# caspervdw/clustertracking

Measured on AMD Instinct MI355X. Metric: cluster-fits/sec, higher is better.
Workload: dtype f64

## Files before the change

clustertracking_amd/_lib.py:

```python
import collections
import contextlib
import ctypes as C
import os
import threading

from . import _abi

_HERE = os.path.dirname(os.path.abspath(__file__))
LIB_PATH = os.environ.get('CTREFINE_LIB') or os.path.join(_HERE, 'csrc', 'libctrefine.so')

_P = C.POINTER
_H = _S = C.c_void_p


def _stage(desc):
    return (C.c_int, [_H, _P(desc), _S])


SIGNATURES = {
    'ctr_abi_version': (C.c_int, []),
    'ctr_create': (C.c_int, [_P(C.c_void_p), C.c_int]),
    'ctr_destroy': (None, [_H]),
    'ctr_last_error': (C.c_char_p, [_H]),
    'ctr_validate_problem': (C.c_int, [_P(_abi.Problem), C.c_char_p, C.c_int]),
    'ctr_cluster_n_vars': (C.c_int, [_P(_abi.Problem), C.c_int]),
    'ctr_cluster_kernel': (C.c_int, [_P(_abi.Problem), C.c_int64, _P(_abi.KernelChoice)]),
    'ctr_refine_batch': (C.c_int, [_H, _P(_abi.Problem), _P(_abi.Batch)]),
    'ctr_plan_create': (C.c_int, [_H, _P(_abi.Problem), C.c_int64, C.c_void_p, _P(C.c_void_p)]),
    'ctr_plan_destroy': (None, [C.c_void_p]),
    'ctr_plan_tail': (C.c_int, [C.c_void_p, _P(C.c_int32), _P(C.c_int32), _P(C.c_int32)]),
    'ctr_refine_batch_device': (C.c_int, [_H, C.c_void_p, _P(_abi.Batch), _S]),
    'ctr_frame_max_device': (C.c_int, [_H, C.c_void_p, C.c_int32, C.c_int64, C.c_int64, C.c_void_p, _S]),
    'ctr_synchronize': (C.c_int, [_H, _S]),
    'ctr_last_kernel_ms': (C.c_int, [_H, _P(C.c_double), _P(C.c_double)]),
    'ctr_find_clusters': (C.c_int, [_H, C.c_int32, C.c_void_p, C.c_void_p, C.c_int64, C.c_void_p,
                                    C.c_void_p, C.c_void_p]),
    'ctr_engine_wait_stream': (C.c_int, [_H, _S]),
    'ctr_stream_wait_engine': (C.c_int, [_H, _S]),
    'ctr_draw_frames_device': (C.c_int, [_H, _P(_abi.Synth), C.c_void_p, _S]),
    'ctr_locate_maxima_device': _stage(_abi.Locate),
    'ctr_characterize_device': _stage(_abi.Characterize),
    'ctr_link_device': _stage(_abi.Link),
    'ctr_preprocess_device': _stage(_abi.Preprocess),
    'ctr_orientation_device': _stage(_abi.Orientation),
    'ctr_diffusion_device': _stage(_abi.Diffusion),
    'ctr_relocate_device': _stage(_abi.Relocate),
    'ctr_relocate_plan': (C.c_int, [_P(_abi.Relocate), _P(C.c_int64), _P(C.c_int64)]),
    'ctr_find_link_device': _stage(_abi.FindLink),
    'ctr_refine_com_device': _stage(_abi.RefineCom),
    'ctr_train_device': _stage(_abi.Train),
    'ctr_cluster_tracks_device': _stage(_abi.ClusterTracks),
    'ctr_cluster_tracks_plan': (C.c_int, [_P(_abi.ClusterTracks), _P(C.c_int64), _P(C.c_int32), _P(C.c_int32)]),
    'ctr_track_positions_device': _stage(_abi.TrackPositions),
    'ctr_drift_device': _stage(_abi.Drift),
    'ctr_drift_subtract_device': _stage(_abi.DriftSubtract),
    'ctr_filter_stubs_device': _stage(_abi.FilterStubs),
    'ctr_msd_device': _stage(_abi.Msd),
    'ctr_emsd_device': _stage(_abi.Emsd),
    'ctr_vanhove_device': _stage(_abi.Vanhove),
    'ctr_pair_correlation_device': _stage(_abi.PairCorrelation),
    'ctr_neighbors_device': _stage(_abi.Neighbors),
    'ctr_twopoint_device': _stage(_abi.TwoPoint),
    'ctr_shape_device': _stage(_abi.Shape),
    'ctr_shape_dynamics_device': _stage(_abi.ShapeDynamics),
    'ctr_shape_plan': (C.c_int, [_P(_abi.ShapeDynamics), _P(C.c_int32), _P(C.c_int32), _P(C.c_int64), _P(C.c_int64),
                                 _P(C.c_int64)]),
    'ctr_shape_histogram_device': _stage(_abi.ShapeHistogram),
    'ctr_residual_device': _stage(_abi.Residual),
    'ctr_residual_plan': (C.c_int, [_P(_abi.Residual), _P(C.c_int32), _P(C.c_int32), _P(C.c_int64), _P(C.c_int64),
                                    _P(C.c_int64), _P(C.c_int64)]),
    'ctr_fit_error_device': _stage(_abi.FitError),
    'ctr_fit_error_plan': (C.c_int, [_P(_abi.FitError), _P(C.c_int32), _P(C.c_int32), _P(C.c_int64), _P(C.c_int64),
                                     _P(C.c_int64)]),
    'ctr_contacts_device': _stage(_abi.Contacts),
    'ctr_contacts_plan': (C.c_int, [_P(_abi.Contacts), _P(C.c_int64), _P(C.c_int64), _P(C.c_int64)]),
    'ctr_refine_prepare_device': _stage(_abi.RefinePrepare),
    'ctr_refine_prepare_plan': (C.c_int, [_P(_abi.RefinePrepare), _P(C.c_int64)]),
    'ctr_find_link_refine_device': (C.c_int, [_H, _P(_abi.FindLink), _P(_abi.RefineCom), _S]),
    'ctr_diffusion_ci_device': _stage(_abi.DiffusionCI),
    'ctr_diffusion_ci_plan': (C.c_int, [_P(_abi.DiffusionCI), _P(C.c_int32), _P(C.c_int64), _P(C.c_int64),
                                        _P(C.c_int64)]),
    'ctr_set_stage_max_grid': (C.c_int32, [_H, C.c_int32]),
    'ctr_set_lane_limit': (C.c_int32, [C.c_int32, C.c_int32]),
# ... 135 lines not shown
    return ContactsPlan(scratch.value, tuple(tiles), tuple(grids))


def refine_prepare_plan(desc):
    return _plan('ctr_refine_prepare_plan', desc, C.c_int64())[0]


class Engine(object):

    def __init__(self, device=0):
        self._lib = load()
        self._h = C.c_void_p()
        rc = self._lib.ctr_create(C.byref(self._h), int(device))
        if rc != _abi.OK:
            msg = self._lib.ctr_last_error(None)
            self._h = None
            raise EngineError("ctr_create(device=%d) failed (%d): %s" % (
                device, rc, (msg or b'').decode()))
        self.device = int(device)

    def close(self):
        if getattr(self, '_h', None):
            self._lib.ctr_destroy(self._h)
            self._h = None

    __del__ = close

    def _check(self, rc, what, too_large=False):
        if rc != _abi.OK:
            msg = (self._lib.ctr_last_error(self._h) or b'').decode()
            if rc == _abi.ERR_INVALID:
                raise ValueError("%s: %s" % (what, msg))
            if rc == _abi.ERR_UNSUPPORTED and too_large:
                raise EngineError("%s: %s" % (what, msg))
            if rc == _abi.ERR_UNSUPPORTED:
                raise NotImplementedError("%s: %s" % (what, msg))
            raise EngineError("%s failed (%d): %s" % (what, rc, msg))

    def refine_batch(self, problem, batch):
        b = batch.as_struct()
        self._check(self._lib.ctr_refine_batch(self._h, C.byref(problem), C.byref(b)),
                    'ctr_refine_batch')
        return batch

    def plan(self, problem, feat_offset_host):
        import numpy as np
        off = np.ascontiguousarray(feat_offset_host, dtype=np.int32)
        plan = C.c_void_p()
        self._check(self._lib.ctr_plan_create(self._h, C.byref(problem), len(off) - 1,
                                              off.ctypes.data, C.byref(plan)),
                    'ctr_plan_create')
        return Plan(self._lib, plan)

    def refine_batch_device(self, plan, batch_struct, stream=None):
        self._check(self._lib.ctr_refine_batch_device(
            self._h, plan._p, C.byref(batch_struct), C.c_void_p(stream or 0)),
            'ctr_refine_batch_device')

    def frame_max_device(self, frames_ptr, dtype_code, n_frames, frame_elems, out_ptr,
                         stream=None):
        self._check(self._lib.ctr_frame_max_device(
            self._h, C.c_void_p(frames_ptr), dtype_code, n_frames, frame_elems,
            C.c_void_p(out_ptr), C.c_void_p(stream or 0)), 'ctr_frame_max_device')

    def find_clusters(self, pos, frame_offset, separation):
        import numpy as np
        pos = np.ascontiguousarray(pos, dtype=np.float64)
        off = np.ascontiguousarray(frame_offset, dtype=np.int32)
        sep = np.ascontiguousarray(separation, dtype=np.float64)
        n, nd = pos.shape
        labels = np.empty(n, dtype=np.int32)
        sizes = np.empty(n, dtype=np.int32)
        self._check(self._lib.ctr_find_clusters(self._h, nd, pos.ctypes.data, off.ctypes.data,
                                                len(off) - 1, sep.ctypes.data,
                                                labels.ctypes.data, sizes.ctypes.data),
                    'ctr_find_clusters')
        return labels, sizes

    def draw_frames_device(self, synth, frames_ptr, stream=None):
        self._check(self._lib.ctr_draw_frames_device(self._h, C.byref(synth), C.c_void_p(frames_ptr),
                                                     C.c_void_p(stream or 0)), 'ctr_draw_frames_device')

    def query_done(self):
        rc = self._lib.ctr_query_done(self._h)
        if rc < 0:
            raise EngineError("ctr_query_done failed: %s" % (self._lib.ctr_last_error(self._h) or b'').decode())
        return rc == 1

    def set_stage_max_grid(self, max_grid):
        return int(self._lib.ctr_set_stage_max_grid(self._h, C.c_int32(int(max_grid))))

    @contextlib.contextmanager
    def stage_max_grid(self, max_grid):
        before = self.set_stage_max_grid(max_grid)
        if before < 0:
            raise ValueError("stage_max_grid: %r is outside [0, 65536]" % (max_grid,))
        try:
            yield self
        finally:
            self.set_stage_max_grid(before)

    def set_lane_limit(self, n):
        return int(self._lib.ctr_set_lane_limit(C.c_int32(self.device), C.c_int32(int(n))))

    def synchronize(self, stream=None):
        self._check(self._lib.ctr_synchronize(self._h, C.c_void_p(stream or 0)),
# ... 65 lines not shown
    method.__doc__ = "``%s``: ``desc`` is its ``_abi`` descriptor with device pointers." % symbol
    return method


for _name, _symbol, _too_large in (
        ('locate_maxima_device', 'ctr_locate_maxima_device', True),
        ('characterize_device', 'ctr_characterize_device', False),
        ('link_device', 'ctr_link_device', False),
        ('preprocess_device', 'ctr_preprocess_device', True),
        ('orientation_device', 'ctr_orientation_device', False),
        ('diffusion_device', 'ctr_diffusion_device', False),
        ('diffusion_ci_device', 'ctr_diffusion_ci_device', False),
        ('relocate_device', 'ctr_relocate_device', False),
        ('find_link_device', 'ctr_find_link_device', False),
        ('refine_com_device', 'ctr_refine_com_device', False),
        ('train_device', 'ctr_train_device', False),
        ('cluster_tracks_device', 'ctr_cluster_tracks_device', False),
        ('track_positions_device', 'ctr_track_positions_device', False),
        ('drift_device', 'ctr_drift_device', False),
        ('drift_subtract_device', 'ctr_drift_subtract_device', False),
        ('filter_stubs_device', 'ctr_filter_stubs_device', False),
        ('msd_device', 'ctr_msd_device', False),
        ('emsd_device', 'ctr_emsd_device', False),
        ('vanhove_device', 'ctr_vanhove_device', False),
        ('pair_correlation_device', 'ctr_pair_correlation_device', False),
        ('neighbors_device', 'ctr_neighbors_device', False),
        ('twopoint_device', 'ctr_twopoint_device', False),
        ('shape_device', 'ctr_shape_device', False),
        ('shape_dynamics_device', 'ctr_shape_dynamics_device', False),
        ('shape_histogram_device', 'ctr_shape_histogram_device', False),
        ('residual_device', 'ctr_residual_device', False),
        ('contacts_device', 'ctr_contacts_device', False),
        ('fit_error_device', 'ctr_fit_error_device', False),
        ('refine_prepare_device', 'ctr_refine_prepare_device', False)):
    setattr(Engine, _name, _stage_method(_symbol, _too_large))


class Plan(object):
    def __init__(self, lib, p):
        self._lib, self._p = lib, p

    def close(self):
        if self._p:
            self._lib.ctr_plan_destroy(self._p)
            self._p = None

    def tail(self):
        fused, cap, grid = C.c_int32(), C.c_int32(), C.c_int32()
        rc = self._lib.ctr_plan_tail(self._p, C.byref(fused), C.byref(cap), C.byref(grid))
        if rc != _abi.OK:
            raise ValueError("ctr_plan_tail: no plan (%d)" % rc)
        return bool(fused.value), int(cap.value), int(grid.value)

    __del__ = close


_default_engines = {}


def default_engine(device=0):
    eng = _default_engines.get(device)
    if eng is None:
        eng = _default_engines[device] = Engine(device)
    return eng
```

clustertracking_amd/csrc/ctrefine.hip:

```cpp
#include <hip/hip_runtime.h>

#include <cmath>
#include <cstdio>
#include <cstdlib>
#include <cstring>
#include <algorithm>
#include <chrono>
#include <functional>
#include <map>
#include <mutex>
#include <string>
#include <vector>

#include "kargs.h"
#include "lane_sched.h"

namespace {

#include "device_common.h"
#include "stage_common.h"
#include "aux_kernels.h"
#include "synth_kernels.h"


std::string g_create_error;
std::mutex g_mutex;

}

constexpr int BIN_TOO_LARGE = MAXNT, BIN_SMALL1 = MAXNT + 1, BIN_SMALL2 = MAXNT + 2, BIN_LARGE = MAXNT + 3,
              BIN_CONS1 = MAXNT + 4, BIN_CONS2 = MAXNT + 5, NBINS = MAXNT + 6;
static_assert(NBINS <= 16, "FrontArgs (aux_kernels.h) holds 16 bins");
constexpr int NFAM = CTR_KFAM_LARGE_LOWPASS + 1, NSLOT = MAXNT + 2;
constexpr int SLOT_SINGLES8 = 0, SLOT_SINGLES64 = 1, SLOT_PAIRS64 = 2, SLOT_PAIRS16 = 3;
constexpr int64_t NARROW_WINDOW = 600;
constexpr int GATE_US = 20;
constexpr int LAUNCH_PAIRS16 = NBINS, LAUNCH_TAIL = NBINS + 1, NLAUNCH = NBINS + 2;
constexpr int TAIL_CAP = 256;
constexpr int TAIL_BINS[TAIL_SEGMENTS] = {BIN_SMALL2, 0, 1};

constexpr int TIMING_EVERY = 8;
struct LaunchTiming {
  lane_sched::Estimate est;
  hipEvent_t t0 = nullptr, t1 = nullptr;
  bool pending = false;
  int untimed = 0;
};

struct ctr_plan {
  ctr_problem prob;
  int64_t n_clusters = 0;
  int device = 0;
  int32_t* d_order = nullptr;
  int* d_front = nullptr;
  double* d_ws = nullptr;
  long long* d_ws_off = nullptr;
  mutable int large_epoch = 0;
  mutable LaunchTiming timing[NLAUNCH];
  int64_t bin_begin[NBINS + 1] = {0};
  int64_t bin_count[NBINS] = {0};
  int32_t bin_family[NBINS] = {0};
  int32_t bin_slot[NBINS] = {0};
  bool gate = false;
  bool pairs_split = false;
  bool tail_fused = false;
  int tail_grid = 0;
  int large_workgroups = 0;
  bool lowpass = false;
  double* d_lp_w = nullptr;
  int lp_half[3] = {0, 0, 0};
};

struct Scratch {
  void* ptr = nullptr;
  size_t bytes = 0;
  hipEvent_t event = nullptr;
};

struct LanePool {
  int device = 0, refs = 0;
  std::mutex mu;
  std::vector<hipStream_t> lanes;
  lane_sched::Pool books;
  std::vector<hipEvent_t> spare;
  explicit LanePool(int n) : books(n) {}
};

struct ctr_handle {
  int device = 0;
  hipStream_t stream = nullptr;
  LanePool* pool = nullptr;
  bool pending = false;
  bool own_dirty = false;
  hipEvent_t ev[4] = {nullptr, nullptr, nullptr, nullptr};
  bool ev_valid = false;
  std::string err;
  Scratch buf, enc, fmax;
  struct { KernelInfo k; bool attr_set; } kernels[NFAM][2][2][NSLOT] = {};
  KernelInfo tail[2] = {};
  bool tail_attr_set[2] = {false, false};
  hipEvent_t ev_done = nullptr;
  hipEvent_t ev_fork = nullptr, ev_gate = nullptr, ev_order = nullptr, ev_own = nullptr;
  int* d_counter = nullptr;
  Scratch link, motion;
  Scratch train;
  Scratch tracks;
  Scratch prepare;
  Scratch drift;
  Scratch msd;
  Scratch pcf;
  Scratch nbr;
  Scratch twopt;
  Scratch shape;
  Scratch resid;
  Scratch contacts;
  Scratch fiterr;
  unsigned stage_max_grid = STAGE_MAX_GRID;
};

namespace {

int fail(ctr_handle* h, int code, const std::string& msg) {
  if (h) h->err = msg;
  else { std::lock_guard<std::mutex> g(g_mutex); g_create_error = msg; }
  return code;
}

#define HIP_TRY(h, call)                                                                   \
  do {                                                                                     \
    hipError_t e_ = (call);                                                                \
    if (e_ != hipSuccess)                                                                  \
      return fail(h, CTR_ERR_DEVICE, std::string(#call) + ": " + hipGetErrorString(e_));   \
  } while (0)

std::map<int, LanePool*> g_pools;
std::mutex g_pool_mutex;

constexpr unsigned PROBE_US = 1000;
bool on_new_queue(const std::vector<hipStream_t>& lanes, hipStream_t cand) {
  for (int rep = 0; rep < 3; ++rep) {
    for (hipStream_t st : lanes) (void)hipStreamSynchronize(st);
    (void)hipStreamSynchronize(cand);
    for (hipStream_t st : lanes) hipLaunchKernelGGL(delay_kernel, dim3(1), dim3(WAVE), 0, st, (unsigned long long)PROBE_US * 100ull);
    const auto t0 = std::chrono::steady_clock::now();
    hipLaunchKernelGGL(delay_kernel, dim3(1), dim3(WAVE), 0, cand, (unsigned long long)PROBE_US * 100ull);
    bool ok = hipGetLastError() == hipSuccess;
    ok = hipStreamSynchronize(cand) == hipSuccess && ok;
    const double us = std::chrono::duration<double, std::micro>(std::chrono::steady_clock::now() - t0).count();
    for (hipStream_t st : lanes) ok = hipStreamSynchronize(st) == hipSuccess && ok;
    if (!ok) return true;
    if (us < 1.5 * PROBE_US) return true;
  }
  return false;
// ... 393 lines not shown
  std::string msg;
  int rc = validate(p, msg);
  if (rc) return fail(h, rc, msg);
  if (n_clusters < 0 || (n_clusters > 0 && !feat_offset_host)) return fail(h, CTR_ERR_INVALID, "bad cluster table");
  if (n_clusters > 0x7ffffff0LL) return fail(h, CTR_ERR_INVALID, "too many clusters for one batch");
  std::vector<int32_t> bin_of((size_t)n_clusters);
  ctr_plan* plan = new ctr_plan();
  plan->prob = *p;
  plan->n_clusters = n_clusters;
  plan->device = h->device;
  plan->lowpass = lowpass_of(p);
  std::vector<long long> ws_off((size_t)n_clusters, 0);
  long long ws_total = 0;
  const long long box_cap = window_volume(p);
  int npf = 0, nsh = 0;
  for (int k2 = 0; k2 < p->n_params; ++k2) {
    if (p->modes[k2] == CTR_MODE_VAR) ++npf;
    else if (p->modes[k2] != CTR_MODE_CONST) ++nsh;
  }
  for (int64_t c = 0; c < n_clusters; ++c) {
    const int64_t n = (int64_t)feat_offset_host[c + 1] - feat_offset_host[c];
    if (n < 0) { delete plan; return fail(h, CTR_ERR_INVALID, "feat_offset must be non-decreasing"); }
    const KernelChoice kc = choose_kernel(p, n);
    const int bin = kc.bin;
    if (bin == BIN_LARGE) {
      ws_off[(size_t)c] = ws_total;
      ws_total += large_ws((int)n, npf, nsh, box_cap).total;
    }
    if (plan->bin_count[bin] == 0) { plan->bin_family[bin] = kc.family; plan->bin_slot[bin] = kc.slot; }
    else if (plan->bin_family[bin] != kc.family || plan->bin_slot[bin] != kc.slot) {
      delete plan;
      return fail(h, CTR_ERR_INVALID, "internal: clusters of one bin with different kernels");
    }
    bin_of[(size_t)c] = bin;
    plan->bin_count[bin]++;
  }
  plan->bin_begin[0] = 0;
  for (int b = 0; b < NBINS; ++b) plan->bin_begin[b + 1] = plan->bin_begin[b] + plan->bin_count[b];
  const bool throughput = (p->flags & CTR_FLAG_THROUGHPUT) != 0;
  plan->gate = n_clusters > plan->bin_count[BIN_SMALL1] + plan->bin_count[BIN_SMALL2] + plan->bin_count[BIN_TOO_LARGE];
  plan->pairs_split = throughput && plan->bin_count[BIN_SMALL2] >= 64 && box_cap <= NARROW_WINDOW;
  {
    int nonempty = 0;
    bool family_ok = true;
    for (int sgm = 0; sgm < TAIL_SEGMENTS; ++sgm) {
      const int bin = TAIL_BINS[sgm];
      if (plan->bin_count[bin] == 0) continue;
      ++nonempty;
      if (bin < MAXNT && plan->bin_family[bin] != CTR_KFAM_GAUSS_TP) family_ok = false;
      plan->tail_grid += (int)std::min<int64_t>(plan->bin_count[bin], TAIL_CAP);
    }
    plan->tail_fused = throughput && p->ndim == 2 && !plan->lowpass && family_ok && nonempty >= 2;
    if (!plan->tail_fused) plan->tail_grid = 0;
  }
  if (plan->bin_count[BIN_LARGE] > 0) {
    const int64_t per_cluster = 512 / plan->bin_count[BIN_LARGE];
    plan->large_workgroups = throughput ? 1 : (int)(per_cluster < 1 ? 1 : (per_cluster > 8 ? 8 : per_cluster));
  }
  std::vector<int32_t> order((size_t)n_clusters);
  {
    int64_t cursor[NBINS];
    for (int b = 0; b < NBINS; ++b) cursor[b] = plan->bin_begin[b];
    for (int64_t c = 0; c < n_clusters; ++c) order[(size_t)cursor[bin_of[(size_t)c]]++] = (int32_t)c;
    for (int b = 0; b < MAXNT; ++b)
      std::stable_sort(order.begin() + plan->bin_begin[b], order.begin() + plan->bin_begin[b + 1],
                       [&](int32_t x, int32_t y) {
                         return feat_offset_host[x + 1] - feat_offset_host[x] > feat_offset_host[y + 1] - feat_offset_host[y];
                       });
  }
  if (n_clusters > 0) {
    if (hipSetDevice(h->device) != hipSuccess ||
        hipMalloc((void**)&plan->d_order, sizeof(int32_t) * 2 * (size_t)n_clusters) != hipSuccess ||
        hipMalloc((void**)&plan->d_front, sizeof(int) * 2 * NBINS) != hipSuccess) {
      ctr_plan_destroy(plan);
      return fail(h, CTR_ERR_NOMEM, "cannot allocate the plan on the device");
    }
    if (hipMemcpy(plan->d_order, order.data(), sizeof(int32_t) * (size_t)n_clusters, hipMemcpyHostToDevice) != hipSuccess) {
      ctr_plan_destroy(plan);
      return fail(h, CTR_ERR_DEVICE, "cannot upload the plan");
    }
    if (plan->lowpass) {
      std::vector<double> taps(3 * LP_STRIDE, 0.);
      for (int a = 0; a < p->ndim; ++a) {
        if (p->noise_size[a] > 0.) plan->lp_half[a] = gaussian_taps(p->noise_size[a], taps.data() + a * LP_STRIDE);
        else taps[(size_t)a * LP_STRIDE] = 1.;
      }
      if (hipMalloc((void**)&plan->d_lp_w, sizeof(double) * taps.size()) != hipSuccess ||
          hipMemcpy(plan->d_lp_w, taps.data(), sizeof(double) * taps.size(), hipMemcpyHostToDevice) != hipSuccess) {
        ctr_plan_destroy(plan);
        return fail(h, CTR_ERR_NOMEM, "cannot upload the lowpass taps");
      }
    }
    if (ws_total > 0) {
      if (hipMalloc((void**)&plan->d_ws, sizeof(double) * (size_t)ws_total) != hipSuccess ||
          hipMalloc((void**)&plan->d_ws_off, sizeof(long long) * (size_t)n_clusters) != hipSuccess) {
        ctr_plan_destroy(plan);
        return fail(h, CTR_ERR_NOMEM, "cannot allocate the workspace of the large clusters on the device");
      }
      if (hipMemset(plan->d_ws, 0, sizeof(double) * (size_t)ws_total) != hipSuccess ||
          hipMemcpy(plan->d_ws_off, ws_off.data(), sizeof(long long) * (size_t)n_clusters, hipMemcpyHostToDevice) != hipSuccess) {
        ctr_plan_destroy(plan);
        return fail(h, CTR_ERR_DEVICE, "cannot upload the plan");
      }
    }
  }
  *out = plan;
  return CTR_OK;
}

void ctr_plan_destroy(ctr_plan* plan) {
  if (!plan) return;
  if (plan->d_order) { (void)hipSetDevice(plan->device); (void)hipFree(plan->d_order); }
  if (plan->d_front) (void)hipFree(plan->d_front);
  if (plan->d_ws) (void)hipFree(plan->d_ws);
  if (plan->d_ws_off) (void)hipFree(plan->d_ws_off);
  if (plan->d_lp_w) (void)hipFree(plan->d_lp_w);
  for (LaunchTiming& t : plan->timing) {
    if (t.t0) (void)hipEventDestroy(t.t0);
    if (t.t1) (void)hipEventDestroy(t.t1);
  }
  delete plan;
}

int ctr_plan_tail(const ctr_plan* plan, int32_t* fused, int32_t* cap, int32_t* tail_grid) {
  if (!plan) return CTR_ERR_INVALID;
  if (fused) *fused = plan->tail_fused ? 1 : 0;
  if (cap) *cap = TAIL_CAP;
  if (tail_grid) *tail_grid = plan->tail_grid;
  return CTR_OK;
}

int ctr_frame_max_device(ctr_handle* h, const void* frames, int32_t frame_dtype, int64_t n_frames,
                         int64_t frame_elems, double* out_max, void* hip_stream) {
  if (!h) return CTR_ERR_INVALID;
  HIP_TRY(h, hipSetDevice(h->device));
  hipStream_t s = hip_stream ? (hipStream_t)hip_stream : own_stream(h);
  return launch_frame_max(h, frames, frame_dtype, n_frames, frame_elems, out_max, s);
}

int ctr_refine_batch_device(ctr_handle* h, const ctr_plan* plan, const ctr_batch* b, void* hip_stream) {
  if (!h || !plan || !b) return CTR_ERR_INVALID;
  if (b->n_clusters != plan->n_clusters) return fail(h, CTR_ERR_INVALID, "batch does not match the plan");
  const ctr_problem& p = plan->prob;
  if (!host_dtype_size(b->frame_dtype)) return fail(h, CTR_ERR_INVALID, "unknown frame dtype");
  for (int a = 0; a < p.ndim; ++a)
    if (b->shape[a] < 1) return fail(h, CTR_ERR_INVALID, "frame shape must be positive");
  HIP_TRY(h, hipSetDevice(h->device));
  const bool own = hip_stream == nullptr;
  LanePool* const pool = h->pool;
  int64_t frame_elems = 1;
  for (int a = 0; a < p.ndim; ++a) frame_elems *= b->shape[a];
  h->ev_valid = false;
  int rc = ensure_fmax(h, b->n_frames > 0 ? b->n_frames : 1);
  if (rc) return rc;

  constexpr double LARGE_CG_TOL2_FAR = 1e-12, LARGE_CG_TOL2_NEAR = 1e-22;
  KArgs k;
  std::memset(&k, 0, sizeof k);
  k.prob = p;
  k.frames = b->frames;
  k.frame_dtype = b->frame_dtype;
  for (int a = 0; a < 3; ++a) k.shape[a] = a < p.ndim ? b->shape[a] : 1;
  k.frame_elems = frame_elems;
  k.frame_index = b->frame_index;
  k.feat_offset = b->feat_offset;
  k.params = b->params;
  k.low = b->low;
  k.high = b->high;
  k.params_out = b->params_out;
  k.cost = b->cost;
  k.status = b->status;
  k.n_rounds = b->n_rounds;
  k.n_iter = b->n_iter;
  k.params_std = b->params_std;
  k.fmax = (const double*)h->fmax.ptr;
  k.lp_w = plan->lowpass ? plan->d_lp_w : nullptr;
  k.cg_tol2_far = LARGE_CG_TOL2_FAR;
  k.cg_tol2_near = LARGE_CG_TOL2_NEAR;
  for (int a = 0; a < 3; ++a) k.lp_half[a] = plan->lp_half[a];
  const int ii = p.isotropic ? 1 : 0;
  std::lock_guard<std::mutex> lock(pool->mu);
  int32_t* ord = plan->d_order + plan->n_clusters;
  struct Chain {
    int launch;
    bool gated;
    std::function<hipError_t(hipStream_t)> run;
  };
  std::vector<Chain> chains;
  auto guess = [&](int launch, lane_sched::ChainClass cls, int64_t count, int nt) {
    plan->timing[launch].est.guess = lane_sched::static_guess(cls, count, nt);
  };
  for (int i = 0; i < MAXNT + 2; ++i) {
    const int bin = i < MAXNT ? MAXNT - 1 - i : (i == MAXNT ? BIN_CONS2 : BIN_CONS1);
    const int64_t cnt = plan->bin_count[bin];
    if (cnt == 0) continue;
    const KernelInfo* ki;
    rc = table_kernel(h, plan->bin_family[bin], p.ndim, ii, plan->bin_slot[bin], &ki);
    if (rc) return rc;
    k.order = ord + plan->bin_begin[bin];
    k.n_bin = (int32_t)cnt;
    const bool in_tail = plan->tail_fused && (bin == TAIL_BINS[1] || bin == TAIL_BINS[2]);
    k.split = in_tail ? plan->d_front + 2 * bin : nullptr;
    k.split_cap = in_tail ? TAIL_CAP : 0;
    guess(bin, lane_sched::CHAIN_BLOCK, cnt, bin < MAXNT ? bin + 1 : (bin == BIN_CONS2 ? 2 : 1));
    chains.push_back({bin, false, [k, ki, cnt](hipStream_t st) {
      void* kargs[] = {(void*)&k};
      return hipLaunchKernel(ki->fn, dim3((unsigned)cnt), dim3((unsigned)ki->threads), kargs, ki->smem, st);
    }});
    k.split = nullptr;
    k.split_cap = 0;
  }
  if (plan->tail_fused) {
    const KernelInfo* ki = &h->tail[ii];
    if (!ki->fn) return fail(h, CTR_ERR_DEVICE, "no tail kernel instantiated for this problem");
    if (!h->tail_attr_set[ii]) {
      HIP_TRY(h, hipFuncSetAttribute(ki->fn, hipFuncAttributeMaxDynamicSharedMemorySize, (int)ki->smem));
      h->tail_attr_set[ii] = true;
    }
    TailArgs ta;
    std::memset(&ta, 0, sizeof ta);
    ta.cap = TAIL_CAP;
    for (int sgm = 0; sgm < TAIL_SEGMENTS; ++sgm) {
      const int bin = TAIL_BINS[sgm];
      const int64_t cnt = plan->bin_count[bin];
      ta.close[sgm] = cnt > 0 ? plan->d_front + 2 * bin : nullptr;
      ta.ord_off[sgm] = (int32_t)plan->bin_begin[bin];
      ta.grid_begin[sgm + 1] = ta.grid_begin[sgm] + (int32_t)std::min<int64_t>(cnt, TAIL_CAP);
    }
    const unsigned grid = (unsigned)plan->tail_grid;
    int* counter = h->d_counter + 4;
    k.order = ord;
    k.n_bin = 0;
    guess(LAUNCH_TAIL, lane_sched::CHAIN_TAIL, (int64_t)grid, 1);
    chains.push_back({LAUNCH_TAIL, false, [k, ki, ta, grid, counter](hipStream_t st) {
      void* kargs[] = {(void*)&k, (void*)&ta, (void*)&counter};
      return hipLaunchKernel(ki->fn, dim3(grid), dim3((unsigned)ki->threads), kargs, ki->smem, st);
    }});
  }
  if (plan->bin_count[BIN_LARGE] > 0) {
    const int64_t cnt = plan->bin_count[BIN_LARGE];
    const KernelInfo* ki;
    rc = table_kernel(h, plan->bin_family[BIN_LARGE], p.ndim, ii, plan->bin_slot[BIN_LARGE], &ki);
    if (rc) return rc;
    k.order = ord + plan->bin_begin[BIN_LARGE];
    k.n_bin = (int32_t)cnt;
    double* wsp = plan->d_ws;
    const long long* wso = plan->d_ws_off;
    int epoch = ++plan->large_epoch;
    const unsigned grid = (unsigned)(cnt * plan->large_workgroups);
    guess(BIN_LARGE, lane_sched::CHAIN_LARGE, cnt, 1);
    chains.push_back({BIN_LARGE, false, [k, ki, grid, wsp, wso, epoch](hipStream_t st) {
      void* kargs[] = {(void*)&k, (void*)&wsp, (void*)&wso, (void*)&epoch};
      return hipLaunchKernel(ki->fn, dim3(grid), dim3((unsigned)ki->threads), kargs, ki->smem, st);
    }});
  }
  if (plan->bin_count[BIN_TOO_LARGE] > 0) {
    const int64_t cnt = plan->bin_count[BIN_TOO_LARGE];
    k.order = ord + plan->bin_begin[BIN_TOO_LARGE];
    k.n_bin = (int32_t)cnt;
    guess(BIN_TOO_LARGE, lane_sched::CHAIN_MARK, cnt, 1);
    chains.push_back({BIN_TOO_LARGE, false, [k, cnt](hipStream_t st) {
      hipLaunchKernelGGL(mark_kernel, dim3((unsigned)((cnt + 255) / 256)), dim3(256), 0, st, k, (int)CTR_STATUS_TOO_LARGE);
      return hipGetLastError();
    }});
  }
  if (plan->bin_count[BIN_SMALL2] > 0) {
    const int64_t cnt = plan->bin_count[BIN_SMALL2];
    const KernelInfo* ki;
    rc = table_kernel(h, plan->bin_family[BIN_SMALL2], p.ndim, ii, plan->bin_slot[BIN_SMALL2], &ki);
    if (rc) return rc;
    int* counter = h->d_counter + 2;
    k.order = ord + plan->bin_begin[BIN_SMALL2];
    k.n_bin = (int32_t)cnt;
    int64_t waves = cnt;
    bool launch64 = true;
    if (plan->tail_fused) {
      k.split = plan->d_front + 2 * BIN_SMALL2;
      k.split_cap = TAIL_CAP;
      k.split_part = 3;
      if (plan->pairs_split) {
        launch64 = cnt > TAIL_CAP;
        waves = std::max<int64_t>(cnt - TAIL_CAP, 1);
      }
    }
    if (plan->pairs_split) {
      const KernelInfo* kb;
      rc = table_kernel(h, plan->bin_family[BIN_SMALL2], p.ndim, ii, SLOT_PAIRS16, &kb);
      if (rc) return rc;
      k.split = plan->d_front + 2 * BIN_SMALL2;
      int* cbulk = h->d_counter + 3;
      k.split_part = 2;
      int64_t wb = (cnt + 3) / 4;
      if (wb > 8192) wb = 8192;
      guess(LAUNCH_PAIRS16, lane_sched::CHAIN_PAIRS16, cnt, 1);
      chains.push_back({LAUNCH_PAIRS16, plan->gate, [k, kb, wb, cbulk](hipStream_t st) {
        hipLaunchKernelGGL(delay_kernel, dim3(1), dim3(WAVE), 0, st, (unsigned long long)GATE_US * 100ull);
        void* kargs[] = {(void*)&k, (void*)&cbulk};
        return hipLaunchKernel(kb->fn, dim3((unsigned)wb), dim3(WAVE), kargs, 0, st);
      }});
      k.split_part = 1;
      if (waves > 2048) waves = 2048;
    }
    if (waves > 8192) waves = 8192;
    guess(BIN_SMALL2, lane_sched::CHAIN_PAIRS64, cnt, 1);
    if (launch64)
      chains.push_back({BIN_SMALL2, plan->gate, [k, ki, waves, counter](hipStream_t st) {
        void* kargs[] = {(void*)&k, (void*)&counter};
        return hipLaunchKernel(ki->fn, dim3((unsigned)waves), dim3(WAVE), kargs, 0, st);
      }});
    k.split = nullptr;
    k.split_part = 0;
    k.split_cap = 0;
  }
  if (plan->bin_count[BIN_SMALL1] > 0) {
    const int64_t cnt = plan->bin_count[BIN_SMALL1];
    const KernelInfo* ki;
    rc = table_kernel(h, plan->bin_family[BIN_SMALL1], p.ndim, ii, plan->bin_slot[BIN_SMALL1], &ki);
    if (rc) return rc;
    int* counter = h->d_counter + 1;
    k.order = ord + plan->bin_begin[BIN_SMALL1];
    k.n_bin = (int32_t)cnt;
    int64_t waves = plan->bin_slot[BIN_SMALL1] == SLOT_SINGLES64 ? cnt : (cnt + 7) / 8;
    if (waves > 8192) waves = 8192;
    guess(BIN_SMALL1, lane_sched::CHAIN_SINGLES, cnt, 1);
    chains.push_back({BIN_SMALL1, plan->gate, [k, ki, waves, counter](hipStream_t st) {
      void* kargs[] = {(void*)&k, (void*)&counter};
      return hipLaunchKernel(ki->fn, dim3((unsigned)waves), dim3(WAVE), kargs, 0, st);
    }});
  }

  lane_sched::Pool& books = pool->books;
  {
    std::vector<lane_sched::EventId> retired;
    books.retire(ticket_done, nullptr, &retired);
    for (lane_sched::EventId ev : retired) pool->spare.push_back((hipEvent_t)ev);
  }
  std::vector<double> est(chains.size());
  for (size_t i = 0; i < chains.size(); ++i) {
    LaunchTiming& t = plan->timing[chains[i].launch];
    if (t.pending && hipEventQuery(t.t1) != hipErrorNotReady) {
      float ms = 0.f;
      if (hipEventElapsedTime(&ms, t.t0, t.t1) == hipSuccess) t.est.update((double)ms);
      t.pending = false;
    }
    est[i] = t.est.value();
  }
  (void)hipGetLastError();
  const double head_ms = lane_sched::static_guess(lane_sched::CHAIN_HEAD, 0);
  const lane_sched::Pool::Placement place = books.place(own ? head_ms : -1., est);

  hipStream_t s = own ? pool->lanes[(size_t)place.head] : (hipStream_t)hip_stream;
  HIP_TRY(h, hipStreamWaitEvent(s, h->ev_done, 0));
  if (own) {
    if (h->own_dirty) {
      HIP_TRY(h, hipEventRecord(h->ev_own, h->stream));
      HIP_TRY(h, hipStreamWaitEvent(s, h->ev_own, 0));
    }
// ... 647 lines not shown
```

clustertracking_amd/csrc/kargs.h:

```cpp
#ifndef CTREFINE_KARGS_H
#define CTREFINE_KARGS_H

#include <hip/hip_runtime.h>

#include <cstddef>
#include <cstdint>

#include "ctrefine.h"

struct KArgs {
  ctr_problem prob;
  const void* frames;
  int32_t frame_dtype;
  int32_t n_bin;
  int64_t shape[3];
  int64_t frame_elems;
  const int32_t* frame_index;
  const int32_t* feat_offset;
  const double* params;
  const double* low;
  const double* high;
  double* params_out;
  double* cost;
  int32_t* status;
  int32_t* n_rounds;
  int32_t* n_iter;
  double* params_std;
  const double* fmax;
  const int32_t* order;
  const int32_t* split;
  int32_t split_part;
  int32_t split_cap;
  int32_t lp_half[3];
  const double* lp_w;
  double cg_tol2_far, cg_tol2_near;
};

constexpr int LP_STRIDE = 40;

constexpr int TAIL_SEGMENTS = 3;
struct TailArgs {
  const int32_t* close[TAIL_SEGMENTS];
  int32_t ord_off[TAIL_SEGMENTS];
  int32_t grid_begin[TAIL_SEGMENTS + 1];
  int32_t cap;
};

struct KernelInfo {
  const void* fn;
  size_t smem;
  int threads;
};

constexpr int LARGE_MAXNB = 48;
constexpr int LARGE_AGG = 4;
constexpr int LARGE_AGG_TRI = 416;
constexpr int LARGE_AGG_STRIDE = 1280;

struct LargeWs {
  long long nvp, nvp_i;
  long long o_vec, o_cur, o_mco, o_fpar, o_pre, o_uq, o_tile, o_off, o_offc, o_int, o_sync, o_pre2, o_agg, o_pix, o_pixv, cap, total;
};

__host__ __device__ inline LargeWs large_ws(int n, int npf, int ns, long long cap) {
  LargeWs W;
  const long long nn = n, nv = ns + nn * npf;
  W.nvp = (nv + 7) & ~7LL;
  W.nvp_i = (nn + 7) & ~7LL;
  long long o = 0;
  W.o_vec = o;  o += 14 * W.nvp;
  W.o_cur = o;  o += W.nvp_i * CTR_MAX_PARAMS;
  W.o_mco = o;  o += W.nvp_i * 3 + 8;
  W.o_fpar = o; o += W.nvp_i * 14;
  W.o_pre = o;  o += W.nvp_i * 32;
  W.o_uq = o;   o += W.nvp_i * 16;
  W.o_tile = o; o += 2 * nn * 256;
  W.o_off = o;  o += 2 * nn * LARGE_MAXNB * 64;
  W.o_offc = o; o += nn * LARGE_MAXNB * npf * npf;
  W.o_int = o;  o += (W.nvp_i + 2 * nn * LARGE_MAXNB + 1) / 2 + 8;
  W.o_pre2 = o; o += (nn / 2 + 1) * LARGE_AGG_STRIDE;
  W.o_agg = o;  o += (3 * W.nvp_i + 4 * (nn / 2 + 1) + 8 + 16 * (nn / 2 + 1) + 1) / 2 + 8;
  W.cap = (cap + 63) & ~63LL;
  W.o_pixv = o; o += nn * W.cap;
  W.o_pix = o;  o += (W.nvp_i + 5 * nn * W.cap + 2 * nn * LARGE_MAXNB + 1) / 2 + 8;
  o = (o + 15) & ~15LL;
  W.o_sync = o; o += 64;
  W.total = (o + 31) & ~31LL;
  return W;
}

KernelInfo ctr_block_kernel_2d(int family, int ndim, int iso, int nt, int cons);
KernelInfo ctr_block_kernel_3d(int family, int ndim, int iso, int nt, int cons);
KernelInfo ctr_block_kernel_lp(int family, int ndim, int iso, int nt, int cons);
KernelInfo ctr_block_kernel_fit2d(int family, int ndim, int iso, int nt, int cons);
KernelInfo ctr_block_kernel_fit3d(int family, int ndim, int iso, int nt, int cons);
KernelInfo ctr_block_kernel_inv(int family, int ndim, int iso, int nt, int cons);
const void* ctr_small_kernel(int ndim, int nf, int iso, int sg);
KernelInfo ctr_tail_kernel(int ndim, int iso);
// ... 84 lines not shown
```

clustertracking_amd/csrc/tail_kernel.h:

```cpp
#ifndef CTREFINE_TAIL_KERNEL_H
#define CTREFINE_TAIL_KERNEL_H

template <int ND>
struct SmemT {
  static constexpr size_t b1 = SmemB<1, 2, false>::bytes, b2 = SmemB<2, 2, false>::bytes,
                          bs = sizeof(double) * SmemS<ND, 2, 64>::total;
  static constexpr size_t bytes = b1 > b2 ? (b1 > bs ? b1 : bs) : (b2 > bs ? b2 : bs);
};

template <int ND, bool ISO>
__global__ void __launch_bounds__(2 * WAVE, 1) refine_tail_kernel(const KArgs k, const TailArgs t, int* __restrict__ counter) {
  extern __shared__ double smem[];
  const int b = (int)blockIdx.x;
  const int seg = b >= t.grid_begin[2] ? 2 : (b >= t.grid_begin[1] ? 1 : 0);
  const int32_t* close = seg == 2 ? t.close[2] : (seg == 1 ? t.close[1] : t.close[0]);
  const int begin = seg == 2 ? t.grid_begin[2] : (seg == 1 ? t.grid_begin[1] : t.grid_begin[0]);
  const int off = seg == 2 ? t.ord_off[2] : (seg == 1 ? t.ord_off[1] : t.ord_off[0]);
  if (close == nullptr) return;
  const int n_close = *close;
  const int count = n_close < t.cap ? n_close : t.cap;
  const int idx = b - begin;
  if (idx >= count) return;
  const int tid = (int)threadIdx.x;
  if (seg == 0) {
    if (tid >= WAVE) return;
    constexpr int NF = 2, SG = 64;
    const int lane = tid;
    double* const lds = smem;
    const int32_t* const order = k.order + off;
    const int id_begin = 0, id_end = count;
#include "small_kernel_body.inc"
  } else if (seg == 1) {
    constexpr int NT = 1, W = 2, FIT = CTR_FIT_GAUSS;
    constexpr bool CONS = false, LP = false;
    const int cl = k.order[off + idx];
#include "block_kernel_body.inc"
  } else {
    constexpr int NT = 2, W = 2, FIT = CTR_FIT_GAUSS;
    constexpr bool CONS = false, LP = false;
    const int cl = k.order[off + idx];
#include "block_kernel_body.inc"
  }
}

#endif
```

include/ctrefine.h:

```cpp
#ifndef CTREFINE_H
#define CTREFINE_H

#include <stdint.h>

#ifdef __cplusplus
extern "C" {
#endif

#define CTR_ABI_VERSION 8
#define CTR_MAX_NDIM 3
#define CTR_MAX_PARAMS 12
#define CTR_MAX_VARS 127
#define CTR_MAX_NEIGHBOURS 48
#define CTR_MAX_NOISE_SIZE 4.0

enum {
  CTR_OK = 0,
  CTR_ERR_INVALID = 1,
  CTR_ERR_UNSUPPORTED = 2,
  CTR_ERR_DEVICE = 3,
  CTR_ERR_NOMEM = 4
};

enum {
// ... 52 lines not shown
  int64_t n_clusters;
  int64_t n_features;
  const int32_t* frame_index;
  const int32_t* feat_offset;
  const double* params;
  const double* low;
  const double* high;
  double* params_out;
  double* cost;
  int32_t* status;
  int32_t* n_rounds;
  int32_t* n_iter;
  double* params_std;
  double* result_rows;
  int64_t* done_flag;
  int64_t done_value;
} ctr_batch;

typedef struct ctr_handle ctr_handle;
typedef struct ctr_plan ctr_plan;

int ctr_abi_version(void);

int ctr_create(ctr_handle** out, int device);
void ctr_destroy(ctr_handle* h);

const char* ctr_last_error(const ctr_handle* h);

int ctr_validate_problem(const ctr_problem* p, char* msg, int msg_len);

int ctr_cluster_n_vars(const ctr_problem* p, int n_features);

enum { CTR_KBIN_SMALL1 = 1, CTR_KBIN_SMALL2 = 2, CTR_KBIN_BLOCK = 3, CTR_KBIN_CONS = 4,
       CTR_KBIN_LARGE = 5, CTR_KBIN_TOO_LARGE = 6 };
enum { CTR_KFAM_NONE = 0, CTR_KFAM_SMALL = 1, CTR_KFAM_GAUSS = 2, CTR_KFAM_GAUSS_TP = 3,
       CTR_KFAM_LOWPASS = 4, CTR_KFAM_RING = 5, CTR_KFAM_DISC = 6, CTR_KFAM_INV_SERIES = 7,
       CTR_KFAM_LARGE = 8, CTR_KFAM_LARGE_LOWPASS = 9 };
typedef struct ctr_kernel_choice {
  int32_t bin;
  int32_t family;
  int32_t nt;
  int32_t lanes;
  int32_t n_vars;
  int32_t reserved0;
} ctr_kernel_choice;
int ctr_cluster_kernel(const ctr_problem* p, int64_t n_features, ctr_kernel_choice* out);

int ctr_refine_batch(ctr_handle* h, const ctr_problem* p, const ctr_batch* b);

int ctr_plan_create(ctr_handle* h, const ctr_problem* p, int64_t n_clusters,
                    const int32_t* feat_offset_host, ctr_plan** out);
void ctr_plan_destroy(ctr_plan* plan);
int ctr_plan_tail(const ctr_plan* plan, int32_t* fused, int32_t* cap, int32_t* tail_grid);
int ctr_refine_batch_device(ctr_handle* h, const ctr_plan* plan,
                            const ctr_batch* b_device, void* hip_stream);

int ctr_frame_max_device(ctr_handle* h, const void* frames, int32_t frame_dtype,
                         int64_t n_frames, int64_t frame_elems, double* out_max,
                         void* hip_stream);

int ctr_find_clusters(ctr_handle* h, int32_t ndim, const double* pos, const int32_t* frame_offset,
                      int64_t n_frames, const double* separation, int32_t* label_out, int32_t* size_out);

typedef struct ctr_synth {
  int32_t ndim;
  int32_t frame_dtype;
  int64_t n_frames;
  int64_t shape[CTR_MAX_NDIM];
  int64_t n_features;
  const int32_t* frame_of;
  const double* pos;
  const double* size;
  const double* max_value;
  double noise;
  uint64_t seed;
} ctr_synth;
int ctr_draw_frames_device(ctr_handle* h, const ctr_synth* s, void* frames_out, void* hip_stream);

typedef struct ctr_locate {
  int32_t ndim;
  int32_t frame_dtype;
  int64_t n_frames;
  int64_t shape[CTR_MAX_NDIM];
  double separation[CTR_MAX_NDIM];
  double percentile;
  int64_t margin[CTR_MAX_NDIM];
  int32_t precise;
  int32_t reserved0;
  int64_t capacity;
  const void* frames;
  int64_t* frame_offset;
  int32_t* pos_out;
  int64_t* total;
  double* threshold;
} ctr_locate;
int ctr_locate_maxima_device(ctr_handle* h, const ctr_locate* l, void* hip_stream);

typedef struct ctr_characterize {
  int32_t ndim;
  int32_t frame_dtype;
  int64_t n_frames;
  int64_t shape[CTR_MAX_NDIM];
  int64_t radius[CTR_MAX_NDIM];
  int32_t isotropic;
  int32_t reserved0;
  double scale_factor;
// ... 784 lines not shown
```

Before: 29.04 million.

## Absorb small tail bins wholly into fused tail kernel with atomic work-stealing

The fused tail kernel can now process entire small bins (up to a configurable absorb threshold) instead of only the first TAIL_CAP clusters. Blocks pull cluster indices from an atomic counter in a persistent loop, and the separate per-bin launches for absorbed bins are skipped. The aim is fewer kernel launches and less split bookkeeping for small workloads. In exchange it adds per-item atomic traffic and serialises more work onto a grid capped at TAIL_CAP blocks per segment.

```diff
diff --git a/clustertracking_amd/_lib.py b/clustertracking_amd/_lib.py
--- a/clustertracking_amd/_lib.py
+++ b/clustertracking_amd/_lib.py
@@ -29,6 +29,8 @@
     'ctr_plan_create': (C.c_int, [_H, _P(_abi.Problem), C.c_int64, C.c_void_p, _P(C.c_void_p)]),
     'ctr_plan_destroy': (None, [C.c_void_p]),
     'ctr_plan_tail': (C.c_int, [C.c_void_p, _P(C.c_int32), _P(C.c_int32), _P(C.c_int32)]),
+    'ctr_plan_tail_bins': (C.c_int, [C.c_void_p, _P(C.c_int32), _P(C.c_int32)]),
+    'ctr_set_tail_absorb': (C.c_int32, [_H, C.c_int32]),
     'ctr_refine_batch_device': (C.c_int, [_H, C.c_void_p, _P(_abi.Batch), _S]),
     'ctr_frame_max_device': (C.c_int, [_H, C.c_void_p, C.c_int32, C.c_int64, C.c_int64, C.c_void_p, _S]),
     'ctr_synchronize': (C.c_int, [_H, _S]),
@@ -270,6 +272,9 @@
                     'ctr_plan_create')
         return Plan(self._lib, plan)
 
+    def set_tail_absorb(self, max_count):
+        return int(self._lib.ctr_set_tail_absorb(self._h, int(max_count)))
+
     def refine_batch_device(self, plan, batch_struct, stream=None):
         self._check(self._lib.ctr_refine_batch_device(
             self._h, plan._p, C.byref(batch_struct), C.c_void_p(stream or 0)),
@@ -441,6 +446,13 @@
             raise ValueError("ctr_plan_tail: no plan (%d)" % rc)
         return bool(fused.value), int(cap.value), int(grid.value)
 
+    def tail_bins(self):
+        absorbed, own = (C.c_int32 * 3)(), (C.c_int32 * 3)()
+        rc = self._lib.ctr_plan_tail_bins(self._p, absorbed, own)
+        if rc != _abi.OK:
+            raise ValueError("ctr_plan_tail_bins: no plan (%d)" % rc)
+        return tuple(bool(v) for v in absorbed), tuple(bool(v) for v in own)
+
     __del__ = close
 
 
diff --git a/clustertracking_amd/csrc/ctrefine.hip b/clustertracking_amd/csrc/ctrefine.hip
--- a/clustertracking_amd/csrc/ctrefine.hip
+++ b/clustertracking_amd/csrc/ctrefine.hip
@@ -37,6 +37,8 @@
 constexpr int GATE_US = 20;
 constexpr int LAUNCH_PAIRS16 = NBINS, LAUNCH_TAIL = NBINS + 1, NLAUNCH = NBINS + 2;
 constexpr int TAIL_CAP = 256;
+constexpr int TAIL_ABSORB = 32 * TAIL_CAP;
+constexpr int TAIL_PAIRS_WHOLE = 8 * TAIL_CAP;
 constexpr int TAIL_BINS[TAIL_SEGMENTS] = {BIN_SMALL2, 0, 1};
 
 constexpr int TIMING_EVERY = 8;
@@ -65,6 +67,8 @@
   bool pairs_split = false;
   bool tail_fused = false;
   int tail_grid = 0;
+  bool tail_whole[TAIL_SEGMENTS] = {false, false, false};
+  bool tail_own[TAIL_SEGMENTS] = {false, false, false};
   int large_workgroups = 0;
   bool lowpass = false;
   double* d_lp_w = nullptr;
@@ -99,6 +103,7 @@
   struct { KernelInfo k; bool attr_set; } kernels[NFAM][2][2][NSLOT] = {};
   KernelInfo tail[2] = {};
   bool tail_attr_set[2] = {false, false};
+  int32_t tail_absorb = TAIL_ABSORB;
   hipEvent_t ev_done = nullptr;
   hipEvent_t ev_fork = nullptr, ev_gate = nullptr, ev_order = nullptr, ev_own = nullptr;
   int* d_counter = nullptr;
@@ -598,6 +603,12 @@
     }
     plan->tail_fused = throughput && p->ndim == 2 && !plan->lowpass && family_ok && nonempty >= 2;
     if (!plan->tail_fused) plan->tail_grid = 0;
+    for (int sgm = 0; sgm < TAIL_SEGMENTS; ++sgm) {
+      const int64_t cnt = plan->bin_count[TAIL_BINS[sgm]];
+      const bool whole = sgm == 0 ? !plan->pairs_split && cnt <= TAIL_PAIRS_WHOLE : cnt <= (int64_t)h->tail_absorb;
+      plan->tail_whole[sgm] = plan->tail_fused && cnt > 0 && whole;
+      plan->tail_own[sgm] = cnt > 0 && !(plan->tail_fused && (whole || (sgm == 0 && plan->pairs_split)));
+    }
   }
   if (plan->bin_count[BIN_LARGE] > 0) {
     const int64_t per_cluster = 512 / plan->bin_count[BIN_LARGE];
@@ -674,6 +685,22 @@
   if (cap) *cap = TAIL_CAP;
   if (tail_grid) *tail_grid = plan->tail_grid;
   return CTR_OK;
+}
+
+int ctr_plan_tail_bins(const ctr_plan* plan, int32_t* absorbed, int32_t* own_launch) {
+  if (!plan) return CTR_ERR_INVALID;
+  for (int sgm = 0; sgm < TAIL_SEGMENTS; ++sgm) {
+    if (absorbed) absorbed[sgm] = plan->tail_whole[sgm] ? 1 : 0;
+    if (own_launch) own_launch[sgm] = plan->tail_own[sgm] ? 1 : 0;
+  }
+  return CTR_OK;
+}
+
+int32_t ctr_set_tail_absorb(ctr_handle* h, int32_t max_count) {
+  if (!h) return -1;
+  const int32_t before = h->tail_absorb;
+  if (max_count >= 0) h->tail_absorb = max_count;
+  return before;
 }
 
 int ctr_frame_max_device(ctr_handle* h, const void* frames, int32_t frame_dtype, int64_t n_frames,
@@ -746,8 +773,9 @@
     k.order = ord + plan->bin_begin[bin];
     k.n_bin = (int32_t)cnt;
     const bool in_tail = plan->tail_fused && (bin == TAIL_BINS[1] || bin == TAIL_BINS[2]);
+    if (in_tail && !plan->tail_own[bin == TAIL_BINS[1] ? 1 : 2]) continue;
     k.split = in_tail ? plan->d_front + 2 * bin : nullptr;
-    k.split_cap = in_tail ? TAIL_CAP : 0;
+    k.split_cap = in_tail ? INT32_MAX : 0;
     guess(bin, lane_sched::CHAIN_BLOCK, cnt, bin < MAXNT ? bin + 1 : (bin == BIN_CONS2 ? 2 : 1));
     chains.push_back({bin, false, [k, ki, cnt](hipStream_t st) {
       void* kargs[] = {(void*)&k};
@@ -765,15 +793,19 @@
     }
     TailArgs ta;
     std::memset(&ta, 0, sizeof ta);
-    ta.cap = TAIL_CAP;
-    for (int sgm = 0; sgm < TAIL_SEGMENTS; ++sgm) {
+    int32_t at = 0;
+    for (int sgm : {1, 2, 0}) {
       const int bin = TAIL_BINS[sgm];
       const int64_t cnt = plan->bin_count[bin];
       ta.close[sgm] = cnt > 0 ? plan->d_front + 2 * bin : nullptr;
       ta.ord_off[sgm] = (int32_t)plan->bin_begin[bin];
-      ta.grid_begin[sgm + 1] = ta.grid_begin[sgm] + (int32_t)std::min<int64_t>(cnt, TAIL_CAP);
-    }
+      ta.whole[sgm] = plan->tail_whole[sgm] ? (int32_t)cnt : 0;
+      ta.grid_begin[sgm] = at;
+      at += (int32_t)std::min<int64_t>(cnt, TAIL_CAP);
+    }
+    ta.grid_begin[TAIL_SEGMENTS] = at;
     const unsigned grid = (unsigned)plan->tail_grid;
+    if (at != plan->tail_grid) return fail(h, CTR_ERR_DEVICE, "internal: the tail launch's grid differs from the plan's");
     int* counter = h->d_counter + 4;
     k.order = ord;
     k.n_bin = 0;
@@ -819,15 +851,11 @@
     k.order = ord + plan->bin_begin[BIN_SMALL2];
     k.n_bin = (int32_t)cnt;
     int64_t waves = cnt;
-    bool launch64 = true;
-    if (plan->tail_fused) {
+    const bool launch64 = plan->tail_own[0];
+    if (launch64 && plan->tail_fused) {
       k.split = plan->d_front + 2 * BIN_SMALL2;
-      k.split_cap = TAIL_CAP;
+      k.split_cap = INT32_MAX;
       k.split_part = 3;
-      if (plan->pairs_split) {
-        launch64 = cnt > TAIL_CAP;
-        waves = std::max<int64_t>(cnt - TAIL_CAP, 1);
-      }
     }
     if (plan->pairs_split) {
       const KernelInfo* kb;
@@ -848,7 +876,7 @@
       if (waves > 2048) waves = 2048;
     }
     if (waves > 8192) waves = 8192;
-    guess(BIN_SMALL2, lane_sched::CHAIN_PAIRS64, cnt, 1);
+    if (launch64) guess(BIN_SMALL2, lane_sched::CHAIN_PAIRS64, cnt, 1);
     if (launch64)
       chains.push_back({BIN_SMALL2, plan->gate, [k, ki, waves, counter](hipStream_t st) {
         void* kargs[] = {(void*)&k, (void*)&counter};
diff --git a/clustertracking_amd/csrc/kargs.h b/clustertracking_amd/csrc/kargs.h
--- a/clustertracking_amd/csrc/kargs.h
+++ b/clustertracking_amd/csrc/kargs.h
@@ -43,7 +43,7 @@
   const int32_t* close[TAIL_SEGMENTS];
   int32_t ord_off[TAIL_SEGMENTS];
   int32_t grid_begin[TAIL_SEGMENTS + 1];
-  int32_t cap;
+  int32_t whole[TAIL_SEGMENTS];
 };
 
 struct KernelInfo {
diff --git a/clustertracking_amd/csrc/tail_kernel.h b/clustertracking_amd/csrc/tail_kernel.h
--- a/clustertracking_amd/csrc/tail_kernel.h
+++ b/clustertracking_amd/csrc/tail_kernel.h
@@ -11,16 +11,14 @@
 template <int ND, bool ISO>
 __global__ void __launch_bounds__(2 * WAVE, 1) refine_tail_kernel(const KArgs k, const TailArgs t, int* __restrict__ counter) {
   extern __shared__ double smem[];
+  __shared__ int tail_entry;
   const int b = (int)blockIdx.x;
-  const int seg = b >= t.grid_begin[2] ? 2 : (b >= t.grid_begin[1] ? 1 : 0);
+  const int seg = b >= t.grid_begin[0] ? 0 : (b >= t.grid_begin[2] ? 2 : 1);
   const int32_t* close = seg == 2 ? t.close[2] : (seg == 1 ? t.close[1] : t.close[0]);
-  const int begin = seg == 2 ? t.grid_begin[2] : (seg == 1 ? t.grid_begin[1] : t.grid_begin[0]);
+  const int whole = seg == 2 ? t.whole[2] : (seg == 1 ? t.whole[1] : t.whole[0]);
   const int off = seg == 2 ? t.ord_off[2] : (seg == 1 ? t.ord_off[1] : t.ord_off[0]);
   if (close == nullptr) return;
-  const int n_close = *close;
-  const int count = n_close < t.cap ? n_close : t.cap;
-  const int idx = b - begin;
-  if (idx >= count) return;
+  const int range = whole > 0 ? whole : *close;
   const int tid = (int)threadIdx.x;
   if (seg == 0) {
     if (tid >= WAVE) return;
@@ -28,18 +26,36 @@
     const int lane = tid;
     double* const lds = smem;
     const int32_t* const order = k.order + off;
-    const int id_begin = 0, id_end = count;
+    const int id_begin = 0, id_end = range;
 #include "small_kernel_body.inc"
   } else if (seg == 1) {
     constexpr int NT = 1, W = 2, FIT = CTR_FIT_GAUSS;
     constexpr bool CONS = false, LP = false;
-    const int cl = k.order[off + idx];
+    for (;;) {
+      if (tid == 0) tail_entry = atomicAdd(counter + 1, 1);
+      __syncthreads();
+      const int tail_next = __builtin_amdgcn_readfirstlane(tail_entry);
+      if (tail_next >= range) break;
+      const int cl = k.order[off + tail_next];
+      {
 #include "block_kernel_body.inc"
+      }
+      __syncthreads();
+    }
   } else {
     constexpr int NT = 2, W = 2, FIT = CTR_FIT_GAUSS;
     constexpr bool CONS = false, LP = false;
-    const int cl = k.order[off + idx];
+    for (;;) {
+      if (tid == 0) tail_entry = atomicAdd(counter + 2, 1);
+      __syncthreads();
+      const int tail_next = __builtin_amdgcn_readfirstlane(tail_entry);
+      if (tail_next >= range) break;
+      const int cl = k.order[off + tail_next];
+      {
 #include "block_kernel_body.inc"
+      }
+      __syncthreads();
+    }
   }
 }
 
diff --git a/include/ctrefine.h b/include/ctrefine.h
--- a/include/ctrefine.h
+++ b/include/ctrefine.h
@@ -128,6 +128,8 @@
                     const int32_t* feat_offset_host, ctr_plan** out);
 void ctr_plan_destroy(ctr_plan* plan);
 int ctr_plan_tail(const ctr_plan* plan, int32_t* fused, int32_t* cap, int32_t* tail_grid);
+int ctr_plan_tail_bins(const ctr_plan* plan, int32_t absorbed[3], int32_t own_launch[3]);
+int32_t ctr_set_tail_absorb(ctr_handle* h, int32_t max_count);
 int ctr_refine_batch_device(ctr_handle* h, const ctr_plan* plan,
                             const ctr_batch* b_device, void* hip_stream);
 
```

Result: faster. 34.83 million (median of 6 runs) (+19.9%).
